# hangxu0304/DeepReduce

Measured on NVIDIA H100. Metric: ResNet-50 images/sec (whole job, device-timed, max over ranks), higher is better.
Workload: dtype bf16

## Files before the change

deepreduce_b200/models/resnet.py:

```python
from __future__ import annotations

import torch.nn as nn
import torch.nn.functional as F

from .fused_bn import bn_add_relu, bn_bn_add_relu, bn_relu, bn_relu_maxpool


class _BasicCifar(nn.Module):
    def __init__(self, inp, out, stride):
        super().__init__()
        self.conv1 = nn.Conv2d(inp, out, 3, stride, 1, bias=False)
        self.bn1 = nn.BatchNorm2d(out)
        self.conv2 = nn.Conv2d(out, out, 3, 1, 1, bias=False)
        self.bn2 = nn.BatchNorm2d(out)
        self.pad = None
        if stride != 1 or inp != out:
            self.pad = (out - inp, stride)

    def forward(self, x):
        y = F.relu(self.bn1(self.conv1(x)))
        y = self.bn2(self.conv2(y))
        if self.pad is not None:
            extra, s = self.pad
            x = F.pad(x[:, :, ::s, ::s], (0, 0, 0, 0, extra // 2, extra - extra // 2))
# ... 41 lines not shown
            self.downsample = nn.Sequential(nn.Conv2d(inp, out, 1, stride, bias=False), nn.BatchNorm2d(out))

    def forward(self, x, skip=None, fork=False):
        skip = x if skip is None else skip
        xd = None if self.downsample is None else self.downsample[0](skip)
        y = bn_relu(self.conv1(x), self.bn1)
        y = bn_relu(self.conv2(y), self.bn2)
        y = self.conv3(y)
        if xd is None:
            return bn_add_relu(y, self.bn3, skip, fork=fork)
        o = bn_bn_add_relu(y, self.bn3, xd, self.downsample[1])
        return (o, None) if fork else o


class ResNet(nn.Module):
    def __init__(self, blocks=(3, 4, 6, 3), num_classes: int = 1000):
        super().__init__()
        self.conv1 = nn.Conv2d(3, 64, 7, 2, 3, bias=False)
        self.bn1 = nn.BatchNorm2d(64)
        self.maxpool = nn.MaxPool2d(3, 2, 1)
        stages, inp = [], 64
        for i, (n, width) in enumerate(zip(blocks, (64, 128, 256, 512))):
            for j in range(n):
                stride = 2 if (j == 0 and i > 0) else 1
                stages.append(_Bottleneck(inp, width, stride, downsample=(j == 0)))
                inp = width * 4
        self.layers = nn.Sequential(*stages)
        self.fc = nn.Linear(inp, num_classes)
        for m in self.modules():
            if isinstance(m, nn.Conv2d):
                nn.init.kaiming_normal_(m.weight, mode="fan_out", nonlinearity="relu")

    def forward(self, x):
        x, skip = bn_relu_maxpool(self.conv1(x), self.bn1, self.maxpool), None
        for blk in self.layers:
            x, skip = blk(x, skip, fork=True)
        x = F.adaptive_avg_pool2d(x, 1).flatten(1)
        return self.fc(x)


def resnet50(num_classes: int = 1000) -> ResNet:
    return ResNet((3, 4, 6, 3), num_classes)
```

deepreduce_b200/ops/csrc/binding.cpp:

```cpp
#include <ATen/cuda/CUDAContext.h>
#include <c10/cuda/CUDAGuard.h>
#include <c10/cuda/CUDAStream.h>
#include <torch/extension.h>

#include <condition_variable>
#include <deque>
#include <mutex>
#include <thread>

#include "ops.h"

namespace py = pybind11;
using dr::EngineParams;

#define CHECK_CUDA_T(x) TORCH_CHECK((x).is_cuda() && (x).is_contiguous(), #x " must be a contiguous CUDA tensor")

static cudaStream_t cur_stream() { return at::cuda::getCurrentCUDAStream().stream(); }

static void check_last(const char* what) {
  cudaError_t e = cudaGetLastError();
  TORCH_CHECK(e == cudaSuccess, what, ": ", cudaGetErrorString(e));
}

static torch::Tensor bloom_insert(torch::Tensor idx, int64_t k, int64_t m_bits, int64_t seed) {
  CHECK_CUDA_T(idx);
  TORCH_CHECK(idx.scalar_type() == torch::kInt64, "idx must be int64");
  c10::cuda::CUDAGuard g(idx.device());
  const int64_t n_words = (m_bits + 31) / 32;
  auto words = torch::zeros({n_words}, idx.options().dtype(torch::kInt32));
  dr::launch_bloom_insert(idx.data_ptr<int64_t>(), idx.numel(), (uint32_t*)words.data_ptr<int32_t>(), (uint32_t)k,
                          (uint32_t)m_bits, (uint32_t)seed, cur_stream());
  check_last("bloom_insert");
  return words;
}

static torch::Tensor bloom_select(torch::Tensor words, int64_t d, int64_t limit, int64_t k, int64_t m_bits, int64_t seed) {
  CHECK_CUDA_T(words);
  c10::cuda::CUDAGuard g(words.device());
  const int64_t n_tiles = (d + dr::kTile - 1) / dr::kTile;
// ... 178 lines not shown

static torch::Tensor u8_to_nhwc_norm(torch::Tensor in, std::vector<double> mean, std::vector<double> stdv) {
  CHECK_CUDA_T(in);
  TORCH_CHECK(in.scalar_type() == torch::kUInt8 && in.size(-1) == 3, "expect uint8 [...,3] NHWC");
  c10::cuda::CUDAGuard g(in.device());
  auto out = torch::empty(in.sizes(), in.options().dtype(torch::kBFloat16));
  float m[3] = {(float)mean[0], (float)mean[1], (float)mean[2]};
  float s[3] = {(float)(1.0 / stdv[0]), (float)(1.0 / stdv[1]), (float)(1.0 / stdv[2])};
  dr::launch_u8_to_nhwc_norm(in.data_ptr<uint8_t>(), out.data_ptr(), in.numel() / 3, m, s, cur_stream());
  check_last("u8_to_nhwc_norm");
  return out;
}

namespace at::native {
struct Var;
template <typename scalar_t, typename VarTransform>
void batch_norm_stats_channels_last_cuda_template(const at::Tensor& out_mean, const at::Tensor& out_invstd,
                                                   const at::Tensor& input, double epsilon);
}

static void check_bn_input(const torch::Tensor& x) {
  TORCH_CHECK(x.is_cuda() && x.scalar_type() == torch::kBFloat16 && x.dim() == 4 && x.stride(1) == 1 &&
                  x.is_contiguous(at::MemoryFormat::ChannelsLast),
              "bn: x must be a channels_last bf16 CUDA tensor");
  TORCH_CHECK(x.size(1) % 8 == 0 && x.size(1) <= 8192, "bn: channels must be a multiple of 8, at most 8192");
  TORCH_CHECK(x.numel() < std::numeric_limits<int32_t>::max(), "bn: tensor too large for 32-bit indexing");
}

static void check_chan(const torch::Tensor& t, int64_t C, const char* what) {
  TORCH_CHECK(t.is_cuda() && t.scalar_type() == torch::kFloat32 && t.is_contiguous() && t.numel() == C, "bn: ", what,
              " must be a contiguous float32 CUDA tensor of C elements");
}

static std::vector<torch::Tensor> bn_stats(torch::Tensor x, torch::Tensor running_mean, torch::Tensor running_var,
                                           double momentum, double eps, bool torch_kernel) {
  check_bn_input(x);
  const int64_t C = x.size(1);
  check_chan(running_mean, C, "running_mean");
  check_chan(running_var, C, "running_var");
  const int64_t N = x.numel() / C;
  TORCH_CHECK(N > 1, "bn: expected more than 1 value per channel when training");
  c10::cuda::CUDAGuard g(x.device());
  auto opts = x.options().dtype(torch::kFloat32);
  auto mean = torch::empty({C}, opts), invstd = torch::empty({C}, opts);
  const float bessel = static_cast<float>(static_cast<double>(N) / static_cast<double>(N - 1));
  int block_y = 0, grid_y = 0;
  dr::bn_row_tree(N, (int)C, &block_y, &grid_y);
  cudaError_t e;
  if (!torch_kernel && (int64_t)block_y * grid_y <= N) {
    auto staging = grid_y > 1 ? torch::empty({(2 * C + 1) * grid_y}, opts) : torch::Tensor();
    const dr::BnStats s{x.data_ptr(), mean.data_ptr<float>(), invstd.data_ptr<float>(), running_mean.data_ptr<float>(),
                        running_var.data_ptr<float>(), grid_y > 1 ? staging.data_ptr<float>() : nullptr,
                        (float)momentum, bessel, (float)eps};
    e = dr::launch_bn_stats(s, N, (int)C, cur_stream());
  } else {
    at::native::batch_norm_stats_channels_last_cuda_template<c10::BFloat16, at::native::Var>(mean, invstd, x, eps);
    e = dr::launch_bn_update_stats(mean.data_ptr<float>(), invstd.data_ptr<float>(), running_mean.data_ptr<float>(),
                                   running_var.data_ptr<float>(), (int)C, (float)momentum, bessel, (float)eps,
                                   cur_stream());
  }
  TORCH_CHECK(e == cudaSuccess, "bn_stats: ", cudaGetErrorString(e));
  return {mean, invstd};
}

static dr::BnParams bn_params(const std::vector<torch::Tensor>& p, int64_t C) {
  TORCH_CHECK(p.size() == 4, "bn: expected (mean, invstd, weight, bias)");
  const char* names[4] = {"mean", "invstd", "weight", "bias"};
  for (int i = 0; i < 4; ++i) check_chan(p[i], C, names[i]);
  return {p[0].data_ptr<float>(), p[1].data_ptr<float>(), p[2].data_ptr<float>(), p[3].data_ptr<float>()};
}

static void check_like_x(const torch::Tensor& t, const torch::Tensor& x, const char* what) {
  TORCH_CHECK(t.sizes() == x.sizes() && t.strides() == x.strides() && t.scalar_type() == torch::kBFloat16 &&
                  t.device() == x.device(),
              "bn: ", what, " must match x in shape, layout, dtype and device");
}

static std::vector<torch::Tensor> bn_apply(int64_t mode, torch::Tensor x, std::vector<torch::Tensor> p,
                                           c10::optional<torch::Tensor> z, std::vector<torch::Tensor> pz) {
  check_bn_input(x);
  const int64_t C = x.size(1);
  const dr::BnParams px = bn_params(p, C);
  dr::BnParams pzz{};
  const void* zp = nullptr;
  if (mode != 0) {
// ... 360 lines not shown
```

deepreduce_b200/ops/csrc/bn.cu:

```cuda
#include <cuda_bf16.h>

#include <algorithm>

#include "common.cuh"
#include "ops.h"

namespace dr {

namespace {

constexpr int kVec = 8;
constexpr int kApplyThreads = 256;
constexpr int kReduceThreads = 128;

struct ChanParams {
  float m[kVec], inv[kVec], w[kVec], b[kVec];
};

__device__ __forceinline__ void load8(const float* __restrict__ p, float* d) {
  const float4 a = __ldg(reinterpret_cast<const float4*>(p));
  const float4 b = __ldg(reinterpret_cast<const float4*>(p) + 1);
  d[0] = a.x; d[1] = a.y; d[2] = a.z; d[3] = a.w;
  d[4] = b.x; d[5] = b.y; d[6] = b.z; d[7] = b.w;
}
// ... 36 lines not shown
  ChanParams a;
  load_params(px, c, a);
  ChanParams d;
  if (kMode == 2) load_params(pz, c, d);
  const int64_t step = (int64_t)gridDim.x * rows_per_cta;
#pragma unroll 2
  for (int64_t r = (int64_t)blockIdx.x * rows_per_cta + rsub; r < rows; r += step) {
    const int64_t off = r * C + c;
    const uint4 vx = *reinterpret_cast<const uint4*>(x + off);
    uint4 vz = make_uint4(0, 0, 0, 0);
    if (kMode != 0) vz = *reinterpret_cast<const uint4*>(z + off);
    const __nv_bfloat16* hx = reinterpret_cast<const __nv_bfloat16*>(&vx);
    const __nv_bfloat16* hz = reinterpret_cast<const __nv_bfloat16*>(&vz);
    uint4 vo;
    __nv_bfloat16* ho = reinterpret_cast<__nv_bfloat16*>(&vo);
    unsigned bits = 0;
#pragma unroll
    for (int i = 0; i < kVec; ++i) {
      __nv_bfloat16 y = __float2bfloat16_rn(bn_elem(__bfloat162float(hx[i]), a.m[i], a.inv[i], a.w[i], a.b[i]));
      if (kMode != 0) {
        const __nv_bfloat16 s = kMode == 1 ? hz[i]
                                           : __float2bfloat16_rn(bn_elem(__bfloat162float(hz[i]), d.m[i], d.inv[i], d.w[i], d.b[i]));
        y = __float2bfloat16_rn(__fadd_rn(__bfloat162float(y), __bfloat162float(s)));
      }
      ho[i] = relu_bf16(y);
      bits |= (__bfloat162float(ho[i]) <= 0.f ? 0u : 1u) << i;
    }
    *reinterpret_cast<uint4*>(out + off) = vo;
    mask[r * groups + c / kVec] = (uint8_t)bits;
  }
}


__global__ void __launch_bounds__(kApplyThreads) bn_apply_pool_kernel(const __nv_bfloat16* __restrict__ x, BnParams px,
                                                                      __nv_bfloat16* __restrict__ out,
                                                                      uint8_t* __restrict__ codes, int64_t orows,
                                                                      PoolGeom pg, int C) {
  const int groups = C / kVec;
  const int rows_per_cta = blockDim.x / groups;
  const int rsub = threadIdx.x / groups;
  if (rsub >= rows_per_cta) return;
  const int c = (threadIdx.x % groups) * kVec;
  ChanParams a;
  load_params(px, c, a);
  const int64_t step = (int64_t)gridDim.x * rows_per_cta;
  for (int64_t r = (int64_t)blockIdx.x * rows_per_cta + rsub; r < orows; r += step) {
    const int ow = (int)(r % pg.Wo);
    const int64_t t = r / pg.Wo;
    const int oh = (int)(t % pg.Ho);
    const int64_t n = t / pg.Ho;
    const int h0 = 2 * oh - 1, w0 = 2 * ow - 1;
    uint4 v[9];
#pragma unroll
    for (int k = 0; k < 9; ++k) {
      const int ih = h0 + k / 3, iw = w0 + k % 3;
      v[k] = ih >= 0 && ih < pg.H && iw >= 0 && iw < pg.W
                 ? *reinterpret_cast<const uint4*>(x + ((n * pg.H + ih) * pg.W + iw) * C + c)
                 : uint4{};
    }
    __nv_bfloat16 best[kVec];
    unsigned slot[kVec];
#pragma unroll
    for (int i = 0; i < kVec; ++i) {
      best[i] = __float2bfloat16_rn(-INFINITY);
      slot[i] = 0;
    }
#pragma unroll
    for (int k = 0; k < 9; ++k) {
      const int ih = h0 + k / 3, iw = w0 + k % 3;
      if (ih < 0 || ih >= pg.H || iw < 0 || iw >= pg.W) continue;
      const __nv_bfloat16* hx = reinterpret_cast<const __nv_bfloat16*>(&v[k]);
#pragma unroll
      for (int i = 0; i < kVec; ++i) {
        const __nv_bfloat16 y = relu_bf16(__float2bfloat16_rn(bn_elem(__bfloat162float(hx[i]), a.m[i], a.inv[i], a.w[i], a.b[i])));
        const float fy = __bfloat162float(y);
        if (fy > __bfloat162float(best[i]) || isnan(fy)) {
          best[i] = y;
          slot[i] = k;
        }
      }
    }
    uint4 vo;
    __nv_bfloat16* ho = reinterpret_cast<__nv_bfloat16*>(&vo);
    uint2 vc;
    uint8_t* hc = reinterpret_cast<uint8_t*>(&vc);
#pragma unroll
    for (int i = 0; i < kVec; ++i) {
      ho[i] = best[i];
      hc[i] = (uint8_t)(slot[i] | (__bfloat162float(best[i]) <= 0.f ? 0u : 0x80u));
    }
    *reinterpret_cast<uint4*>(out + r * C + c) = vo;
    *reinterpret_cast<uint2*>(codes + r * C + c) = vc;
  }
}

struct PoolGather {
  uint4 g[4];
  uint2 code[4];
  int off;
  int nh, nw;
  int sh, sw;
};

__device__ __forceinline__ void pool_gather_codes(PoolGather& q, const uint8_t* __restrict__ codes, const PoolGeom& pg,
                                                  int row, int C, int c, bool valid) {
  const int w = row % pg.W, t = row / pg.W, h = t % pg.H, n = t / pg.H;
  const int ph = h >> 1, pw = w >> 1;
  q.nh = valid ? min((h + 1) / 2 + 1, pg.Ho) - ph : 0;
  q.nw = valid ? min((w + 1) / 2 + 1, pg.Wo) - pw : 0;
  q.sh = h - 2 * ph + 1;
  q.sw = w - 2 * pw + 1;
  q.off = ((n * pg.Ho + ph) * pg.Wo + pw) * C + c;
#pragma unroll
  for (int k = 0; k < 4; ++k) {
    const int a = k >> 1, b = k & 1;
    q.code[k] = a < q.nh && b < q.nw ? *reinterpret_cast<const uint2*>(codes + q.off + (a * pg.Wo + b) * C) : uint2{};
  }
}

template <bool kTwo>
__device__ __forceinline__ void pool_gather_grads(PoolGather& q, const __nv_bfloat16* __restrict__ gp,
                                                  const __nv_bfloat16* __restrict__ gp2, const PoolGeom& pg, int C) {
#pragma unroll
  for (int k = 0; k < 4; ++k) {
    const int a = k >> 1, b = k & 1;
    const bool in = a < q.nh && b < q.nw;
    const int off = q.off + (a * pg.Wo + b) * C;
    q.g[k] = in ? *reinterpret_cast<const uint4*>(gp + off) : uint4{};
    if (kTwo && in) q.g[k] = add_bf16x8(q.g[k], *reinterpret_cast<const uint4*>(gp2 + off));
  }
}

__device__ __forceinline__ void pool_gather_resolve(const PoolGather& q, uint4& g, unsigned& bits) {
  __nv_bfloat16* hg = reinterpret_cast<__nv_bfloat16*>(&g);
  const bool single = q.nh == 1 && q.nw == 1;
  bits = 0;
#pragma unroll
  for (int i = 0; i < kVec; ++i) {
    float s = 0.f;
    __nv_bfloat16 one = __float2bfloat16_rn(0.f);
    unsigned bit = 0;
#pragma unroll
    for (int k = 0; k < 4; ++k) {
      const int a = k >> 1, b = k & 1;
      const unsigned code = (reinterpret_cast<const uint8_t*>(&q.code[k]))[i];
      if (a < q.nh && b < q.nw && (int)(code & 0x7fu) == (q.sh - 2 * a) * 3 + (q.sw - 2 * b)) {
        const __nv_bfloat16 v = (reinterpret_cast<const __nv_bfloat16*>(&q.g[k]))[i];
        s = __fadd_rn(s, __bfloat162float(v));
        one = v;
        bit = code >> 7;
      }
    }
    hg[i] = single ? one : __float2bfloat16_rn(s);
    bits |= bit << i;
  }
}

template <bool kTwo>
__global__ void __launch_bounds__(kApplyThreads) bn_pool_grad_kernel(const __nv_bfloat16* __restrict__ gp,
                                                                     const __nv_bfloat16* __restrict__ gp2,
                                                                     const uint8_t* __restrict__ codes,
                                                                     __nv_bfloat16* __restrict__ g, PoolGeom pg,
                                                                     int64_t rows, int C) {
  const int groups = C / kVec;
  const int rows_per_cta = blockDim.x / groups;
  const int rsub = threadIdx.x / groups;
  if (rsub >= rows_per_cta) return;
  const int c = (threadIdx.x % groups) * kVec;
  const int64_t step = (int64_t)gridDim.x * rows_per_cta;
#pragma unroll 2
  for (int64_t r = (int64_t)blockIdx.x * rows_per_cta + rsub; r < rows; r += step) {
    PoolGather q;
    pool_gather_codes(q, codes, pg, (int)r, C, c, true);
    pool_gather_grads<kTwo>(q, gp, gp2, pg, C);
    uint4 v;
    unsigned bits;
    pool_gather_resolve(q, v, bits);
    __nv_bfloat16* hv = reinterpret_cast<__nv_bfloat16*>(&v);
#pragma unroll
    for (int i = 0; i < kVec; ++i)
      if (!((bits >> i) & 1u)) hv[i] = __float2bfloat16_rn(0.f);
    *reinterpret_cast<uint4*>(g + r * C + c) = v;
  }
}

struct RowTree {
  int block_y, grid_y;
  __host__ __device__ int S() const { return block_y * grid_y; }
  __host__ __device__ int loops(int rows) const { return 1 + (rows - 1) / (S() * kLoads); }
  static constexpr int kLoads = 4;
};

constexpr int kStatsThreads = 256;

__device__ __forceinline__ void welford_update(float x, float inv, float valid, float& mean, float& m2n) {
  const float d0 = __fsub_rn(x, mean);
  mean = __fmaf_rn(d0, inv, mean);
  const float d1 = __fsub_rn(x, mean);
  m2n = __fmaf_rn(__fmul_rn(d0, d1), valid, m2n);
}

template <int kN, bool kFuseNew>
__device__ __forceinline__ void welford_merge(int& n, float* mean, float* m2n, int n_new, const float* mean_new,
                                              const float* m2n_new) {
  const float fn = (float)n, fn_new = (float)n_new;
  const float factor = __frcp_rn((float)max(1, n + n_new));
#pragma unroll
  for (int i = 0; i < kN; ++i) {
    const float d = __fsub_rn(mean[i], mean_new[i]);
    const float s = kFuseNew ? __fmaf_rn(mean_new[i], fn_new, __fmul_rn(mean[i], fn))
                             : __fmaf_rn(mean[i], fn, __fmul_rn(mean_new[i], fn_new));
    mean[i] = __fmul_rn(s, factor);
    const float u = __fmul_rn(__fmul_rn(__fmul_rn(d, d), fn_new), fn);
    m2n[i] = __fadd_rn(m2n[i], __fmaf_rn(u, factor, m2n_new[i]));
  }
// ... 3 lines not shown
template <int kN>
struct WelfordSlots {
  float* mean; float* m2n; int* count;
  __device__ WelfordSlots(float* sh, int slots)
      : mean(sh), m2n(sh + slots * kN), count(reinterpret_cast<int*>(sh + 2 * slots * kN)) {}
  __device__ void put(int s, int n, const float* m, const float* q) const {
#pragma unroll
    for (int i = 0; i < kN; ++i) { mean[s * kN + i] = m[i]; m2n[s * kN + i] = q[i]; }
    count[s] = n;
  }
  template <bool kFuseNew>
  __device__ void merge_from(int s, int& n, float* m, float* q) const {
    float mn[kN], qn[kN];
#pragma unroll
    for (int i = 0; i < kN; ++i) { mn[i] = mean[s * kN + i]; qn[i] = m2n[s * kN + i]; }
    welford_merge<kN, kFuseNew>(n, m, q, count[s], mn, qn);
  }
  static size_t bytes(int slots) { return (size_t)slots * (2 * kN * sizeof(float) + sizeof(int)); }
};

template <int kN>
__device__ __forceinline__ void welford_tree_over_y(const WelfordSlots<kN>& sl, bool part, int y, int block_y, int base,
                                                    int stride, int& n, float* mean, float* m2n) {
  for (int off = block_y / 2; off > 0; off >>= 1) {
    if (part && y < 2 * off) sl.put(base + y * stride, n, mean, m2n);
    __syncthreads();
    if (part && y < off) sl.template merge_from<false>(base + (y + off) * stride, n, mean, m2n);
    __syncthreads();
  }
}

struct StatsOut {
  float* mean; float* invstd; float* running_mean; float* running_var;
  float* st_mean; float* st_m2n; int* st_count;
  float momentum, bessel, eps;
};

__device__ __forceinline__ void stats_store(const StatsOut& o, int c, int n, float mean, float m2n) {
  const float var = __fdiv_rn(m2n, (float)n);
  const float keep = __fsub_rn(1.f, o.momentum);
  o.mean[c] = mean;
  o.invstd[c] = rsqrtf(__fadd_rn(var, o.eps));
  o.running_mean[c] = __fmaf_rn(mean, o.momentum, __fmul_rn(o.running_mean[c], keep));
  o.running_var[c] = __fmaf_rn(__fmul_rn(var, o.bessel), o.momentum, __fmul_rn(o.running_var[c], keep));
}

__global__ void __launch_bounds__(kStatsThreads) bn_stats_kernel(const __nv_bfloat16* __restrict__ x, StatsOut o,
                                                                 RowTree t, int rows, int C) {
  constexpr int L = RowTree::kLoads;
  constexpr int kAhead = 4;
  extern __shared__ float sh[];
  const int gpc = blockDim.x / (L * t.block_y);
  const int g = threadIdx.x % gpc, j = (threadIdx.x / gpc) % L, y = threadIdx.x / (gpc * L);
  const int group = blockIdx.x * gpc + g;
  const bool live = group * kVec < C;
  const int c = live ? group * kVec : 0;
  const int S = t.S();
  const int n_loops = t.loops(rows);
  const int r0 = blockIdx.y * t.block_y + y + j * S;
  const int rstep = L * S;
  float mean[kVec], m2n[kVec];
#pragma unroll
  for (int i = 0; i < kVec; ++i) mean[i] = m2n[i] = 0.f;
  int n = 0;
  auto load = [&](uint4* b, int i0) {
#pragma unroll
    for (int u = 0; u < kAhead; ++u) {
      const int r = r0 + (i0 + u) * rstep;
      b[u] = live && i0 + u < n_loops && r < rows ? *reinterpret_cast<const uint4*>(x + (size_t)r * C + c) : uint4{};
    }
  };
  uint4 cur[kAhead];
  load(cur, 0);
  for (int i0 = 0; i0 < n_loops; i0 += kAhead) {
    uint4 nxt[kAhead];
    load(nxt, i0 + kAhead);
#pragma unroll
    for (int u = 0; u < kAhead; ++u) {
      const int i = i0 + u;
      if (i >= n_loops) break;
      const bool valid = r0 + i * rstep < rows;
      const float inv = valid ? __frcp_rn((float)(i + 1)) : 0.f;
      const float fv = valid ? 1.f : 0.f;
      n += valid;
      const __nv_bfloat16* hx = reinterpret_cast<const __nv_bfloat16*>(&cur[u]);
#pragma unroll
      for (int k = 0; k < kVec; ++k) welford_update(__bfloat162float(hx[k]), inv, fv, mean[k], m2n[k]);
    }
#pragma unroll
    for (int u = 0; u < kAhead; ++u) cur[u] = nxt[u];
  }
  const WelfordSlots<kVec> sl(sh, blockDim.x);
  sl.put(threadIdx.x, n, mean, m2n);
  __syncthreads();
  if (j == 0) {
#pragma unroll
    for (int a = 1; a < L; ++a) sl.merge_from<true>(threadIdx.x + a * gpc, n, mean, m2n);
  }
  __syncthreads();
  welford_tree_over_y<kVec>(sl, j == 0, y, t.block_y, g, gpc * L, n, mean, m2n);
  if (j != 0 || y != 0 || !live) return;
  if (t.grid_y == 1) {
#pragma unroll
    for (int i = 0; i < kVec; ++i) stats_store(o, c + i, n, mean[i], m2n[i]);
    return;
  }
#pragma unroll
  for (int i = 0; i < kVec; ++i) {
    o.st_mean[(size_t)blockIdx.y * C + c + i] = mean[i];
    o.st_m2n[(size_t)blockIdx.y * C + c + i] = m2n[i];
  }
  if (group == 0) o.st_count[blockIdx.y] = n;
}

__global__ void bn_stats_finalize_kernel(StatsOut o, RowTree t, int C) {
  extern __shared__ float sh[];
  const int cols = blockDim.x / t.block_y;
  const int col = threadIdx.x % cols, y = threadIdx.x / cols;
  const int c = blockIdx.x * cols + col;
  int n = 0;
  float mean = 0.f, m2n = 0.f;
  if (c < C)
    for (int b = y; b < t.grid_y; b += t.block_y) {
      const float mb = o.st_mean[(size_t)b * C + c], qb = o.st_m2n[(size_t)b * C + c];
      welford_merge<1, false>(n, &mean, &m2n, o.st_count[b], &mb, &qb);
    }
  const WelfordSlots<1> sl(sh, blockDim.x);
  welford_tree_over_y<1>(sl, true, y, t.block_y, col, cols, n, &mean, &m2n);
  if (y == 0 && c < C) stats_store(o, c, n, mean, m2n);
}


template <int kN>
__device__ __forceinline__ void tree_over_y(float* v, float* sh, int y, int n, int col, int width) {
  for (int off = n / 2; off > 0; off >>= 1) {
#pragma unroll
    for (int i = 0; i < kN; ++i) sh[y * width + col + i] = v[i];
    __syncthreads();
    if (y < off) {
#pragma unroll
      for (int i = 0; i < kN; ++i) v[i] = __fadd_rn(v[i], sh[(y + off) * width + col + i]);
    }
    __syncthreads();
  }
}

struct BwdOut {
  float* sums;
  float* dw; float* db; float* dwz; float* dbz;
  float* staging;
};

__device__ __forceinline__ void bwd_store(const BwdOut& o, int k, int c, int C, float v, const float* invstd,
                                         const float* invstd_z) {
  o.sums[k * C + c] = v;
  if (k == 0) {
    o.db[c] = v;
    if (o.dbz) o.dbz[c] = v;
  } else if (k == 1) {
    o.dw[c] = __fmul_rn(v, invstd[c]);
  } else {
    o.dwz[c] = __fmul_rn(v, invstd_z[c]);
// ... 195 lines not shown
      if (kMode == 2) hd[i] = elemt(g, __bfloat162float(hz[i]), q, i, norm);
    }
    *reinterpret_cast<uint4*>(dx + off) = vo;
    if (kMode == 2) *reinterpret_cast<uint4*>(dz + off) = vd;
  }
}

__global__ void bn_update_stats_kernel(const float* __restrict__ mean, float* __restrict__ var_invstd,
                                       float* __restrict__ running_mean, float* __restrict__ running_var, int C,
                                       float momentum, float bessel, float eps) {
  const int c = blockIdx.x * blockDim.x + threadIdx.x;
  if (c >= C) return;
  const float m = mean[c], v = var_invstd[c];
  const float unbiased_var = v * bessel;
  running_mean[c] = m * momentum + (1 - momentum) * running_mean[c];
  running_var[c] = unbiased_var * momentum + (1 - momentum) * running_var[c];
  var_invstd[c] = rsqrtf(v + eps);
}

template <typename K>
cudaError_t rows_grid(K kernel, int64_t rows, int C, int& grid, int& threads) {
  const int groups = C / kVec;
  const int rows_per_cta = groups >= kApplyThreads ? 1 : kApplyThreads / groups;
  threads = groups * rows_per_cta;
  int per_sm = 0;
  cudaError_t e = cudaOccupancyMaxActiveBlocksPerMultiprocessor(&per_sm, kernel, threads, 0);
  if (e != cudaSuccess) return e;
  int64_t g = (rows + rows_per_cta - 1) / rows_per_cta;
  const int64_t cap = (int64_t)(per_sm > 0 ? per_sm : 1) * sm_count();
  grid = (int)(g > cap ? cap : g);
  return cudaSuccess;
}

template <int kMode>
cudaError_t launch_apply(const void* x, const BnParams& px, const void* z, const BnParams& pz, void* out, void* mask,
                         int64_t rows, int C, cudaStream_t st) {
  if (rows == 0) return cudaSuccess;
  int grid = 0, threads = 0;
  cudaError_t e = rows_grid(bn_apply_kernel<kMode>, rows, C, grid, threads);
  if (e != cudaSuccess) return e;
  count_launch();
  bn_apply_kernel<kMode><<<grid, threads, 0, st>>>(reinterpret_cast<const __nv_bfloat16*>(x), px,
                                                   reinterpret_cast<const __nv_bfloat16*>(z), pz,
                                                   reinterpret_cast<__nv_bfloat16*>(out),
                                                   reinterpret_cast<uint8_t*>(mask), rows, C);
  return cudaGetLastError();
}

int last_pow2(unsigned n) {
  n |= n >> 1; n |= n >> 2; n |= n >> 4; n |= n >> 8; n |= n >> 16;
  return std::max<int>(1, (int)(n - (n >> 1)));
}

RowTree row_tree(int rows, int C) {
  const int block_x = std::min(last_pow2((unsigned)C), 32);
  const int block_y = std::min(last_pow2((unsigned)((rows + 15) / 16)), 512 / block_x);
  int grid_y = std::min((rows + block_y * 16 - 1) / (block_y * 16), 128);
  if (grid_y < 8) grid_y = 1;
  return {block_y, grid_y};
}

template <int kMode, bool kTwo>
cudaError_t launch_bwd_reduce(const BnBwd& b, const RowTree& t, const BwdOut& o, int rows, int C, cudaStream_t st) {
  const int groups = C / kVec;
  const int gpc = std::min(groups, std::max(1, kReduceThreads / t.block_y));
  const dim3 grid((groups + gpc - 1) / gpc, t.grid_y);
  const int threads = gpc * t.block_y;
  count_launch();
  bn_bwd_reduce_kernel<kMode, kTwo><<<grid, threads, threads * kVec * sizeof(float), st>>>(
      reinterpret_cast<const __nv_bfloat16*>(b.go), reinterpret_cast<const __nv_bfloat16*>(b.go2), b.mask,
      reinterpret_cast<const __nv_bfloat16*>(b.x), b.px.mean, b.px.invstd, reinterpret_cast<const __nv_bfloat16*>(b.z),
      b.pz.mean, b.pz.invstd, reinterpret_cast<__nv_bfloat16*>(b.g), o, t, rows, C);
  return cudaGetLastError();
}

template <int kMode, bool kTwo>
cudaError_t launch_bwd_elemt(const BnBwd& b, const ElemtArgs& a, int64_t rows, int C, cudaStream_t st) {
  int grid = 0, threads = 0;
  cudaError_t e = rows_grid(bn_bwd_elemt_kernel<kMode, kTwo>, rows, C, grid, threads);
  if (e != cudaSuccess) return e;
  const float norm = (float)(1.0 / (double)rows);
  count_launch();
  bn_bwd_elemt_kernel<kMode, kTwo><<<grid, threads, 0, st>>>(
      reinterpret_cast<const __nv_bfloat16*>(kMode == 1 || kMode == 3 ? b.g : b.go),
      reinterpret_cast<const __nv_bfloat16*>(b.go2), b.mask, reinterpret_cast<const __nv_bfloat16*>(b.x),
      reinterpret_cast<const __nv_bfloat16*>(b.z), a, reinterpret_cast<__nv_bfloat16*>(b.dx),
      reinterpret_cast<__nv_bfloat16*>(b.dz), norm, rows, C);
  return cudaGetLastError();
}

template <int kMode, bool kTwo>
cudaError_t launch_backward(const BnBwd& b, int64_t rows64, int C, cudaStream_t st) {
  const int rows = (int)rows64;
  const RowTree t = row_tree(rows, C);
  const BwdOut o{b.sums, b.dw, b.db, b.dwz, b.dbz, b.staging};
  cudaError_t e;
  if (kMode == 3) {
    int grid = 0, threads = 0;
    e = rows_grid(bn_pool_grad_kernel<kTwo>, rows64, C, grid, threads);
    if (e != cudaSuccess) return e;
    count_launch();
    bn_pool_grad_kernel<kTwo><<<grid, threads, 0, st>>>(reinterpret_cast<const __nv_bfloat16*>(b.go),
                                                        reinterpret_cast<const __nv_bfloat16*>(b.go2), b.mask,
                                                        reinterpret_cast<__nv_bfloat16*>(b.g), b.pool, rows64, C);
    e = cudaGetLastError();
    if (e != cudaSuccess) return e;
  }
  BnBwd bb = b;
  if (kMode == 3) bb.go = b.g;
  e = launch_bwd_reduce<kMode, kTwo && kMode != 3>(bb, t, o, rows, C, st);
  if (e != cudaSuccess) return e;
  if (t.grid_y > 1) {
    const int cols = std::max(1, 512 / t.block_y);
    const int threads = cols * t.block_y;
    count_launch();
    bn_bwd_finalize_kernel<<<(C + cols - 1) / cols, threads, threads * sizeof(float), st>>>(
        o, t, kMode == 2 ? 3 : 2, C, b.px.invstd, b.pz.invstd);
    e = cudaGetLastError();
    if (e != cudaSuccess) return e;
  }
  const ElemtArgs a{b.px.mean, b.px.invstd, b.px.weight, b.sums, b.pz.mean, b.pz.invstd, b.pz.weight};
  return launch_bwd_elemt<kMode, kTwo && kMode == 2>(b, a, rows64, C, st);
}

cudaError_t launch_stats(const BnStats& s, int rows, int C, cudaStream_t st) {
  const RowTree t = row_tree(rows, C);
  const int grid_y = t.grid_y;
  const StatsOut o{s.mean, s.invstd, s.running_mean, s.running_var,
                   s.staging, s.staging + (size_t)grid_y * C, reinterpret_cast<int*>(s.staging + 2 * (size_t)grid_y * C),
                   s.momentum, s.bessel, s.eps};
  const int groups = C / kVec;
  const int gpc = std::min(groups, std::max(1, kStatsThreads / (RowTree::kLoads * t.block_y)));
  const int threads = gpc * RowTree::kLoads * t.block_y;
  count_launch();
  bn_stats_kernel<<<dim3((groups + gpc - 1) / gpc, grid_y), threads, WelfordSlots<kVec>::bytes(threads), st>>>(
      reinterpret_cast<const __nv_bfloat16*>(s.x), o, t, rows, C);
  cudaError_t e = cudaGetLastError();
  if (e != cudaSuccess || grid_y == 1) return e;
  const int cols = std::max(1, 512 / t.block_y);
  const int fthreads = cols * t.block_y;
  count_launch();
  bn_stats_finalize_kernel<<<(C + cols - 1) / cols, fthreads, WelfordSlots<1>::bytes(fthreads), st>>>(o, t, C);
  return cudaGetLastError();
}

}

void bn_row_tree(int64_t rows, int C, int* block_y, int* grid_y) {
  const RowTree t = row_tree((int)rows, C);
  *block_y = t.block_y;
  *grid_y = t.grid_y;
}

cudaError_t launch_bn_backward(int mode, const BnBwd& b, int64_t rows, int C, cudaStream_t st) {
  if (rows == 0) return cudaSuccess;
  const bool two = b.go2 != nullptr;
  switch (mode) {
    case 0: return two ? cudaErrorInvalidValue : launch_backward<0, false>(b, rows, C, st);
    case 1: return two ? launch_backward<1, true>(b, rows, C, st) : launch_backward<1, false>(b, rows, C, st);
    case 2: return two ? launch_backward<2, true>(b, rows, C, st) : launch_backward<2, false>(b, rows, C, st);
    case 3: return two ? launch_backward<3, true>(b, rows, C, st) : launch_backward<3, false>(b, rows, C, st);
    default: return cudaErrorInvalidValue;
  }
}

cudaError_t launch_bn_stats(const BnStats& s, int64_t rows, int C, cudaStream_t st) {
  if (rows == 0) return cudaSuccess;
  return launch_stats(s, (int)rows, C, st);
}

cudaError_t launch_bn_update_stats(const float* mean, float* var_invstd, float* running_mean, float* running_var, int C,
                                   float momentum, float bessel, float eps, cudaStream_t st) {
  count_launch();
  bn_update_stats_kernel<<<(C + 255) / 256, 256, 0, st>>>(mean, var_invstd, running_mean, running_var, C, momentum,
                                                          bessel, eps);
  return cudaGetLastError();
}

cudaError_t launch_bn_apply(int mode, const void* x, const BnParams& px, const void* z, const BnParams& pz, void* out,
                            void* mask, int64_t rows, int C, cudaStream_t st) {
  switch (mode) {
    case 0: return launch_apply<0>(x, px, z, pz, out, mask, rows, C, st);
    case 1: return launch_apply<1>(x, px, z, pz, out, mask, rows, C, st);
    case 2: return launch_apply<2>(x, px, z, pz, out, mask, rows, C, st);
    default: return cudaErrorInvalidValue;
  }
}

cudaError_t launch_bn_apply_pool(const void* x, const BnParams& px, void* out, void* codes, int N, const PoolGeom& pg,
                                 int C, cudaStream_t st) {
  const int64_t orows = (int64_t)N * pg.Ho * pg.Wo;
  if (orows == 0) return cudaSuccess;
  int grid = 0, threads = 0;
  cudaError_t e = rows_grid(bn_apply_pool_kernel, orows, C, grid, threads);
  if (e != cudaSuccess) return e;
  count_launch();
  bn_apply_pool_kernel<<<grid, threads, 0, st>>>(reinterpret_cast<const __nv_bfloat16*>(x), px,
                                                 reinterpret_cast<__nv_bfloat16*>(out),
                                                 reinterpret_cast<uint8_t*>(codes), orows, pg, C);
  return cudaGetLastError();
}

}
```

deepreduce_b200/ops/csrc/ops.h:

```cpp
#pragma once
#include <cuda_runtime.h>
#include <stdint.h>

#include "plan.h"

namespace dr {

int engine_max_grid(int blocks_per_sm, int dyn_smem_bytes);
cudaError_t engine_launch(const EngineParams& P, int grid, int blocks_per_sm, int dyn_smem_bytes, cudaStream_t stream);
void count_launch(int n);
long long launch_count();

void launch_bloom_insert(const int64_t* idx, int64_t n, uint32_t* filter, uint32_t n_hash, uint32_t m_bits,
                         uint32_t seed, cudaStream_t st);
void launch_bloom_count(const uint32_t* filter, uint32_t d, uint32_t n_hash, uint32_t m_bits, uint32_t seed,
                        uint32_t* tile_counts, uint32_t* tile_excl, cudaStream_t st);
void launch_bloom_emit(const uint32_t* filter, uint32_t d, uint32_t n_hash, uint32_t m_bits, uint32_t seed,
                       const uint32_t* tile_excl, int64_t* out, uint32_t limit, cudaStream_t st);
void launch_qsgd_encode(const float* v, int64_t K, int bucket, int q, uint32_t seed, void* lvl, bool i16, float* norms,
                        cudaStream_t st);
void launch_qsgd_decode(const void* lvl, bool i16, const float* norms, int64_t K, int bucket, int q, float* out,
                        cudaStream_t st);
void launch_pack_bits(const int64_t* vals, int64_t n, int bits, uint32_t* out, int64_t n_words, cudaStream_t st);
void launch_unpack_bits(const uint32_t* in, int64_t n_words, int64_t n, int bits, int64_t* out, cudaStream_t st);
void launch_polyfit_fit(const float* y, const int* seg_off, const int* seg_len, int n_seg, int degree, float* coeffs,
                        cudaStream_t st);
void launch_polyfit_eval(const float* coeffs, const int* seg_off, const int* seg_len, int n_seg, int degree,
                         int64_t total, float* out, cudaStream_t st);
cudaError_t launch_conflict_sets_pick(const uint32_t* set_off, const uint32_t* members, uint32_t* last, uint32_t n_sets, uint32_t n_pos,
                                      uint32_t K, uint32_t pseed, uint32_t* chosen_out, cudaStream_t st);
void launch_dexp_fit(const float* y, int64_t K, double* out_abpq, cudaStream_t st);
void launch_bp128_widths(const int64_t* idx, int64_t n, uint32_t* widths, cudaStream_t st);
void launch_bp128_pack(const int64_t* idx, int64_t n, const uint32_t* widths, const int64_t* word_off, uint32_t* out,
                       cudaStream_t st);
void launch_bp128_unpack(const uint32_t* in, int64_t n, int64_t* word_off, int64_t* deltas, cudaStream_t st);
void launch_rle_count(const int64_t* idx, int64_t n, uint32_t* counts, uint32_t* excl, cudaStream_t st);
void launch_rle_runs(const int64_t* idx, int64_t n, const uint32_t* excl, int64_t* start_pos, int64_t* end_pos,
                     int64_t n_runs, int64_t d, int64_t* runs, cudaStream_t st);
void launch_rle_expand(const int64_t* ones_excl, const int64_t* run_start, int64_t n_runs, int64_t total, int64_t* out,
                       cudaStream_t st);

struct ArenaHandle { unsigned char bytes[64]; };
void* arena_alloc(size_t bytes);
void arena_free(void* p);
ArenaHandle arena_export(void* p);
void* arena_import(const ArenaHandle& h);
void arena_close(void* p);
int arena_enable_peer_access(const int* devices, int n);
void launch_u8_to_nhwc_norm(const uint8_t* in, void* out_bf16, int64_t n_pix, const float* mean, const float* inv_std,
                            cudaStream_t st);

struct BnParams { const float* mean; const float* invstd; const float* weight; const float* bias; };
void bn_row_tree(int64_t rows, int C, int* block_y, int* grid_y);
struct BnStats {
  const void* x;
  float* mean; float* invstd; float* running_mean; float* running_var;
  float* staging;
  float momentum, bessel, eps;
};
cudaError_t launch_bn_stats(const BnStats& s, int64_t rows, int C, cudaStream_t st);
cudaError_t launch_bn_update_stats(const float* mean, float* var_invstd, float* running_mean, float* running_var, int C,
                                   float momentum, float bessel, float eps, cudaStream_t st);
cudaError_t launch_bn_apply(int mode, const void* x, const BnParams& px, const void* z, const BnParams& pz, void* out,
                            void* mask, int64_t rows, int C, cudaStream_t st);
struct PoolGeom { int H, W, Ho, Wo; };
cudaError_t launch_bn_apply_pool(const void* x, const BnParams& px, void* out, void* codes, int N, const PoolGeom& pg,
                                 int C, cudaStream_t st);
struct BnBwd {
  const void* go; const void* go2; const uint8_t* mask; const void* x; const void* z;
  BnParams px, pz;
  void* dx; void* dz; void* g;
  float* sums; float* staging; float* dw; float* db; float* dwz; float* dbz;
  PoolGeom pool;
};
cudaError_t launch_bn_backward(int mode, const BnBwd& b, int64_t rows, int C, cudaStream_t st);

}
```

Baseline: 6178.

## Fuse BN stats finalize via last-block reduction and rework maxpool kernels

```diff
diff --git a/deepreduce_b200/models/resnet.py b/deepreduce_b200/models/resnet.py
--- a/deepreduce_b200/models/resnet.py
+++ b/deepreduce_b200/models/resnet.py
@@ -97,7 +97,7 @@
                 nn.init.kaiming_normal_(m.weight, mode="fan_out", nonlinearity="relu")
 
     def forward(self, x):
-        x, skip = bn_relu_maxpool(self.conv1(x), self.bn1, self.maxpool), None
+        x, skip = bn_relu_maxpool(self.conv1(x), self.bn1, self.maxpool, fork=True)
         for blk in self.layers:
             x, skip = blk(x, skip, fork=True)
         x = F.adaptive_avg_pool2d(x, 1).flatten(1)
diff --git a/deepreduce_b200/ops/csrc/binding.cpp b/deepreduce_b200/ops/csrc/binding.cpp
--- a/deepreduce_b200/ops/csrc/binding.cpp
+++ b/deepreduce_b200/ops/csrc/binding.cpp
@@ -5,6 +5,7 @@
 
 #include <condition_variable>
 #include <deque>
+#include <map>
 #include <mutex>
 #include <thread>
 
@@ -249,6 +250,20 @@
               " must be a contiguous float32 CUDA tensor of C elements");
 }
 
+static unsigned* bn_stats_arrivals(int device, cudaStream_t st) {
+  static std::mutex mu;
+  static std::map<std::pair<int, cudaStream_t>, unsigned*> sets;
+  std::lock_guard<std::mutex> lock(mu);
+  unsigned*& p = sets[{device, st}];
+  if (p == nullptr) {
+    void* q = nullptr;
+    C10_CUDA_CHECK(cudaMalloc(&q, dr::kBnStatsArrivals * sizeof(unsigned)));
+    C10_CUDA_CHECK(cudaMemsetAsync(q, 0, dr::kBnStatsArrivals * sizeof(unsigned), st));
+    p = static_cast<unsigned*>(q);
+  }
+  return p;
+}
+
 static std::vector<torch::Tensor> bn_stats(torch::Tensor x, torch::Tensor running_mean, torch::Tensor running_var,
                                            double momentum, double eps, bool torch_kernel) {
   check_bn_input(x);
@@ -265,9 +280,10 @@
   dr::bn_row_tree(N, (int)C, &block_y, &grid_y);
   cudaError_t e;
   if (!torch_kernel && (int64_t)block_y * grid_y <= N) {
-    auto staging = grid_y > 1 ? torch::empty({(2 * C + 1) * grid_y}, opts) : torch::Tensor();
+    auto staging = grid_y > 1 ? torch::empty({(2 * C + C / 8) * grid_y}, opts) : torch::Tensor();
     const dr::BnStats s{x.data_ptr(), mean.data_ptr<float>(), invstd.data_ptr<float>(), running_mean.data_ptr<float>(),
                         running_var.data_ptr<float>(), grid_y > 1 ? staging.data_ptr<float>() : nullptr,
+                        grid_y > 1 ? bn_stats_arrivals(x.get_device(), cur_stream()) : nullptr,
                         (float)momentum, bessel, (float)eps};
     e = dr::launch_bn_stats(s, N, (int)C, cur_stream());
   } else {
diff --git a/deepreduce_b200/ops/csrc/bn.cu b/deepreduce_b200/ops/csrc/bn.cu
--- a/deepreduce_b200/ops/csrc/bn.cu
+++ b/deepreduce_b200/ops/csrc/bn.cu
@@ -92,32 +92,89 @@
 }
 
 
-__global__ void __launch_bounds__(kApplyThreads) bn_apply_pool_kernel(const __nv_bfloat16* __restrict__ x, BnParams px,
-                                                                      __nv_bfloat16* __restrict__ out,
-                                                                      uint8_t* __restrict__ codes, int64_t orows,
-                                                                      PoolGeom pg, int C) {
+constexpr int kPoolThreads = 128;
+constexpr int kPoolWalk = 8;
+
+struct PoolWalk {
+  int64_t n;
+  int oh, ow0, ow1, c;
+};
+
+__device__ __forceinline__ bool pool_walk(const PoolGeom& pg, int N, int C, PoolWalk& w) {
   const int groups = C / kVec;
-  const int rows_per_cta = blockDim.x / groups;
-  const int rsub = threadIdx.x / groups;
-  if (rsub >= rows_per_cta) return;
-  const int c = (threadIdx.x % groups) * kVec;
+  const int segs = (pg.Wo + kPoolWalk - 1) / kPoolWalk;
+  const int64_t t = (int64_t)blockIdx.x * blockDim.x + threadIdx.x;
+  const int64_t task = t / groups;
+  if (task >= (int64_t)N * pg.Ho * segs) return false;
+  w.c = (int)(t % groups) * kVec;
+  const int seg = (int)(task % segs);
+  const int64_t row = task / segs;
+  w.oh = (int)(row % pg.Ho);
+  w.n = row / pg.Ho;
+  w.ow0 = seg * kPoolWalk;
+  w.ow1 = min(w.ow0 + kPoolWalk, pg.Wo);
+  return true;
+}
+
+__device__ __forceinline__ uint4 bn_relu8(const uint4& v, const ChanParams& a) {
+  uint4 r;
+  const __nv_bfloat16* hx = reinterpret_cast<const __nv_bfloat16*>(&v);
+  __nv_bfloat16* hr = reinterpret_cast<__nv_bfloat16*>(&r);
+#pragma unroll
+  for (int i = 0; i < kVec; ++i)
+    hr[i] = relu_bf16(__float2bfloat16_rn(bn_elem(__bfloat162float(hx[i]), a.m[i], a.inv[i], a.w[i], a.b[i])));
+  return r;
+}
+
+__global__ void __launch_bounds__(kPoolThreads) bn_apply_pool_kernel(const __nv_bfloat16* __restrict__ x, BnParams px,
+                                                                     __nv_bfloat16* __restrict__ out,
+                                                                     uint8_t* __restrict__ codes, int N, PoolGeom pg,
+                                                                     int C) {
+  PoolWalk w;
+  if (!pool_walk(pg, N, C, w)) return;
   ChanParams a;
-  load_params(px, c, a);
-  const int64_t step = (int64_t)gridDim.x * rows_per_cta;
-  for (int64_t r = (int64_t)blockIdx.x * rows_per_cta + rsub; r < orows; r += step) {
-    const int ow = (int)(r % pg.Wo);
-    const int64_t t = r / pg.Wo;
-    const int oh = (int)(t % pg.Ho);
-    const int64_t n = t / pg.Ho;
-    const int h0 = 2 * oh - 1, w0 = 2 * ow - 1;
-    uint4 v[9];
-#pragma unroll
-    for (int k = 0; k < 9; ++k) {
-      const int ih = h0 + k / 3, iw = w0 + k % 3;
-      v[k] = ih >= 0 && ih < pg.H && iw >= 0 && iw < pg.W
-                 ? *reinterpret_cast<const uint4*>(x + ((n * pg.H + ih) * pg.W + iw) * C + c)
-                 : uint4{};
-    }
+  load_params(px, w.c, a);
+  bool row_in[3];
+  const __nv_bfloat16* xrow[3];
+#pragma unroll
+  for (int kh = 0; kh < 3; ++kh) {
+    const int ih = 2 * w.oh - 1 + kh;
+    row_in[kh] = ih >= 0 && ih < pg.H;
+    xrow[kh] = x + ((w.n * pg.H + (row_in[kh] ? ih : 0)) * pg.W) * C + w.c;
+  }
+  auto load = [&](int kh, int iw) {
+    return row_in[kh] && iw >= 0 && iw < pg.W ? *reinterpret_cast<const uint4*>(xrow[kh] + (int64_t)iw * C) : uint4{};
+  };
+  uint4 left[3];
+  uint4 nxt[3][2];
+#pragma unroll
+  for (int kh = 0; kh < 3; ++kh) {
+    left[kh] = bn_relu8(load(kh, 2 * w.ow0 - 1), a);
+    nxt[kh][0] = load(kh, 2 * w.ow0);
+    nxt[kh][1] = load(kh, 2 * w.ow0 + 1);
+  }
+  int64_t o = ((w.n * pg.Ho + w.oh) * pg.Wo + w.ow0) * C + w.c;
+  for (int ow = w.ow0; ow < w.ow1; ++ow, o += C) {
+    uint4 v[3][3];
+#pragma unroll
+    for (int kh = 0; kh < 3; ++kh) {
+      v[kh][0] = left[kh];
+      v[kh][1] = nxt[kh][0];
+      v[kh][2] = nxt[kh][1];
+    }
+    if (ow + 1 < w.ow1)
+#pragma unroll
+      for (int kh = 0; kh < 3; ++kh) {
+        nxt[kh][0] = load(kh, 2 * ow + 2);
+        nxt[kh][1] = load(kh, 2 * ow + 3);
+      }
+#pragma unroll
+    for (int kh = 0; kh < 3; ++kh) {
+      v[kh][1] = bn_relu8(v[kh][1], a);
+      v[kh][2] = bn_relu8(v[kh][2], a);
+      left[kh] = v[kh][2];
+    }
+    const bool col_in[3] = {ow > 0, true, 2 * ow + 1 < pg.W};
     __nv_bfloat16 best[kVec];
     unsigned slot[kVec];
 #pragma unroll
@@ -127,15 +184,13 @@
     }
 #pragma unroll
     for (int k = 0; k < 9; ++k) {
-      const int ih = h0 + k / 3, iw = w0 + k % 3;
-      if (ih < 0 || ih >= pg.H || iw < 0 || iw >= pg.W) continue;
-      const __nv_bfloat16* hx = reinterpret_cast<const __nv_bfloat16*>(&v[k]);
+      if (!row_in[k / 3] || !col_in[k % 3]) continue;
+      const __nv_bfloat16* hy = reinterpret_cast<const __nv_bfloat16*>(&v[k / 3][k % 3]);
 #pragma unroll
       for (int i = 0; i < kVec; ++i) {
-        const __nv_bfloat16 y = relu_bf16(__float2bfloat16_rn(bn_elem(__bfloat162float(hx[i]), a.m[i], a.inv[i], a.w[i], a.b[i])));
-        const float fy = __bfloat162float(y);
+        const float fy = __bfloat162float(hy[i]);
         if (fy > __bfloat162float(best[i]) || isnan(fy)) {
-          best[i] = y;
+          best[i] = hy[i];
           slot[i] = k;
         }
       }
@@ -149,47 +204,17 @@
       ho[i] = best[i];
       hc[i] = (uint8_t)(slot[i] | (__bfloat162float(best[i]) <= 0.f ? 0u : 0x80u));
     }
-    *reinterpret_cast<uint4*>(out + r * C + c) = vo;
-    *reinterpret_cast<uint2*>(codes + r * C + c) = vc;
+    *reinterpret_cast<uint4*>(out + o) = vo;
+    *reinterpret_cast<uint2*>(codes + o) = vc;
   }
 }
 
 struct PoolGather {
   uint4 g[4];
   uint2 code[4];
-  int off;
   int nh, nw;
   int sh, sw;
 };
-
-__device__ __forceinline__ void pool_gather_codes(PoolGather& q, const uint8_t* __restrict__ codes, const PoolGeom& pg,
-                                                  int row, int C, int c, bool valid) {
-  const int w = row % pg.W, t = row / pg.W, h = t % pg.H, n = t / pg.H;
-  const int ph = h >> 1, pw = w >> 1;
-  q.nh = valid ? min((h + 1) / 2 + 1, pg.Ho) - ph : 0;
-  q.nw = valid ? min((w + 1) / 2 + 1, pg.Wo) - pw : 0;
-  q.sh = h - 2 * ph + 1;
-  q.sw = w - 2 * pw + 1;
-  q.off = ((n * pg.Ho + ph) * pg.Wo + pw) * C + c;
-#pragma unroll
-  for (int k = 0; k < 4; ++k) {
-    const int a = k >> 1, b = k & 1;
-    q.code[k] = a < q.nh && b < q.nw ? *reinterpret_cast<const uint2*>(codes + q.off + (a * pg.Wo + b) * C) : uint2{};
-  }
-}
-
-template <bool kTwo>
-__device__ __forceinline__ void pool_gather_grads(PoolGather& q, const __nv_bfloat16* __restrict__ gp,
-                                                  const __nv_bfloat16* __restrict__ gp2, const PoolGeom& pg, int C) {
-#pragma unroll
-  for (int k = 0; k < 4; ++k) {
-    const int a = k >> 1, b = k & 1;
-    const bool in = a < q.nh && b < q.nw;
-    const int off = q.off + (a * pg.Wo + b) * C;
-    q.g[k] = in ? *reinterpret_cast<const uint4*>(gp + off) : uint4{};
-    if (kTwo && in) q.g[k] = add_bf16x8(q.g[k], *reinterpret_cast<const uint4*>(gp2 + off));
-  }
-}
 
 __device__ __forceinline__ void pool_gather_resolve(const PoolGather& q, uint4& g, unsigned& bits) {
   __nv_bfloat16* hg = reinterpret_cast<__nv_bfloat16*>(&g);
@@ -217,30 +242,63 @@
 }
 
 template <bool kTwo>
-__global__ void __launch_bounds__(kApplyThreads) bn_pool_grad_kernel(const __nv_bfloat16* __restrict__ gp,
-                                                                     const __nv_bfloat16* __restrict__ gp2,
-                                                                     const uint8_t* __restrict__ codes,
-                                                                     __nv_bfloat16* __restrict__ g, PoolGeom pg,
-                                                                     int64_t rows, int C) {
-  const int groups = C / kVec;
-  const int rows_per_cta = blockDim.x / groups;
-  const int rsub = threadIdx.x / groups;
-  if (rsub >= rows_per_cta) return;
-  const int c = (threadIdx.x % groups) * kVec;
-  const int64_t step = (int64_t)gridDim.x * rows_per_cta;
-#pragma unroll 2
-  for (int64_t r = (int64_t)blockIdx.x * rows_per_cta + rsub; r < rows; r += step) {
-    PoolGather q;
-    pool_gather_codes(q, codes, pg, (int)r, C, c, true);
-    pool_gather_grads<kTwo>(q, gp, gp2, pg, C);
-    uint4 v;
-    unsigned bits;
-    pool_gather_resolve(q, v, bits);
-    __nv_bfloat16* hv = reinterpret_cast<__nv_bfloat16*>(&v);
-#pragma unroll
-    for (int i = 0; i < kVec; ++i)
-      if (!((bits >> i) & 1u)) hv[i] = __float2bfloat16_rn(0.f);
-    *reinterpret_cast<uint4*>(g + r * C + c) = v;
+__global__ void __launch_bounds__(kPoolThreads) bn_pool_grad_kernel(const __nv_bfloat16* __restrict__ gp,
+                                                                    const __nv_bfloat16* __restrict__ gp2,
+                                                                    const uint8_t* __restrict__ codes,
+                                                                    __nv_bfloat16* __restrict__ g, int N, PoolGeom pg,
+                                                                    int C) {
+  PoolWalk w;
+  if (!pool_walk(pg, N, C, w)) return;
+  const int nh = min(2, pg.Ho - w.oh);
+  const int64_t prow = (w.n * pg.Ho + w.oh) * pg.Wo;
+  auto load = [&](int a, int ow, uint4& gv, uint2& cv) {
+    if (a < nh && ow < pg.Wo) {
+      const int64_t off = (prow + (int64_t)a * pg.Wo + ow) * C + w.c;
+      gv = *reinterpret_cast<const uint4*>(gp + off);
+      if (kTwo) gv = add_bf16x8(gv, *reinterpret_cast<const uint4*>(gp2 + off));
+      cv = *reinterpret_cast<const uint2*>(codes + off);
+    } else {
+      gv = uint4{};
+      cv = uint2{};
+    }
+  };
+  uint4 gl[2];
+  uint2 cl[2];
+  load(0, w.ow0, gl[0], cl[0]);
+  load(1, w.ow0, gl[1], cl[1]);
+  for (int ow = w.ow0; ow < w.ow1; ++ow) {
+    uint4 gr[2];
+    uint2 cr[2];
+    load(0, ow + 1, gr[0], cr[0]);
+    load(1, ow + 1, gr[1], cr[1]);
+    const int nw = min(2, pg.Wo - ow);
+#pragma unroll
+    for (int a = 0; a < 2; ++a) {
+      const int h = 2 * w.oh + a;
+      if (h >= pg.H) break;
+#pragma unroll
+      for (int b = 0; b < 2; ++b) {
+        const int iw = 2 * ow + b;
+        if (iw >= pg.W) break;
+        PoolGather q;
+        q.g[0] = gl[0]; q.g[1] = gr[0]; q.g[2] = gl[1]; q.g[3] = gr[1];
+        q.code[0] = cl[0]; q.code[1] = cr[0]; q.code[2] = cl[1]; q.code[3] = cr[1];
+        q.nh = a == 0 ? 1 : nh;
+        q.nw = b == 0 ? 1 : nw;
+        q.sh = a + 1;
+        q.sw = b + 1;
+        uint4 v;
+        unsigned bits;
+        pool_gather_resolve(q, v, bits);
+        __nv_bfloat16* hv = reinterpret_cast<__nv_bfloat16*>(&v);
+#pragma unroll
+        for (int i = 0; i < kVec; ++i)
+          if (!((bits >> i) & 1u)) hv[i] = __float2bfloat16_rn(0.f);
+        *reinterpret_cast<uint4*>(g + ((w.n * pg.H + h) * pg.W + iw) * C + w.c) = v;
+      }
+    }
+    gl[0] = gr[0]; gl[1] = gr[1];
+    cl[0] = cr[0]; cl[1] = cr[1];
   }
 }
 
@@ -310,7 +368,7 @@
 
 struct StatsOut {
   float* mean; float* invstd; float* running_mean; float* running_var;
-  float* st_mean; float* st_m2n; int* st_count;
+  float* st_mean; float* st_m2n; int* st_count; unsigned* arrivals;
   float momentum, bessel, eps;
 };
 
@@ -323,7 +381,44 @@
   o.running_var[c] = __fmaf_rn(__fmul_rn(var, o.bessel), o.momentum, __fmul_rn(o.running_var[c], keep));
 }
 
-__global__ void __launch_bounds__(kStatsThreads) bn_stats_kernel(const __nv_bfloat16* __restrict__ x, StatsOut o,
+__device__ __forceinline__ void stats_cross_block(const StatsOut& o, const RowTree& t, float* sh, int C, int cb_c0) {
+  constexpr int kRows = 8;
+  const int cols = blockDim.x / t.block_y;
+  const int col = threadIdx.x % cols, y = threadIdx.x / cols;
+  const int c = cb_c0 + 2 * col;
+  const bool live = c < C;
+  int n = 0;
+  float mean[2] = {0.f, 0.f}, m2n[2] = {0.f, 0.f};
+  if (live)
+    for (int b0 = y; b0 < t.grid_y; b0 += kRows * t.block_y) {
+      float2 mb[kRows], qb[kRows];
+      int nb[kRows];
+#pragma unroll
+      for (int u = 0; u < kRows; ++u) {
+        const int b = b0 + u * t.block_y;
+        if (b < t.grid_y) {
+          const size_t off = (size_t)b * C + c;
+          mb[u] = __ldcg(reinterpret_cast<const float2*>(o.st_mean + off));
+          qb[u] = __ldcg(reinterpret_cast<const float2*>(o.st_m2n + off));
+          nb[u] = __ldcg(o.st_count + (size_t)blockIdx.x * t.grid_y + b);
+        }
+      }
+#pragma unroll
+      for (int u = 0; u < kRows; ++u) {
+        if (b0 + u * t.block_y >= t.grid_y) break;
+        const float mbv[2] = {mb[u].x, mb[u].y}, qbv[2] = {qb[u].x, qb[u].y};
+        welford_merge<2, false>(n, mean, m2n, nb[u], mbv, qbv);
+      }
+    }
+  const WelfordSlots<2> sl(sh, blockDim.x);
+  welford_tree_over_y<2>(sl, true, y, t.block_y, col, cols, n, mean, m2n);
+  if (y == 0 && live) {
+    stats_store(o, c, n, mean[0], m2n[0]);
+    stats_store(o, c + 1, n, mean[1], m2n[1]);
+  }
+}
+
+__global__ void __launch_bounds__(kStatsThreads, 768 / kStatsThreads) bn_stats_kernel(const __nv_bfloat16* __restrict__ x, StatsOut o,
                                                                  RowTree t, int rows, int C) {
   constexpr int L = RowTree::kLoads;
   constexpr int kAhead = 4;
@@ -377,35 +472,32 @@
   }
   __syncthreads();
   welford_tree_over_y<kVec>(sl, j == 0, y, t.block_y, g, gpc * L, n, mean, m2n);
-  if (j != 0 || y != 0 || !live) return;
+  const bool head = j == 0 && y == 0 && live;
   if (t.grid_y == 1) {
-#pragma unroll
-    for (int i = 0; i < kVec; ++i) stats_store(o, c + i, n, mean[i], m2n[i]);
+    if (head)
+#pragma unroll
+      for (int i = 0; i < kVec; ++i) stats_store(o, c + i, n, mean[i], m2n[i]);
     return;
   }
-#pragma unroll
-  for (int i = 0; i < kVec; ++i) {
-    o.st_mean[(size_t)blockIdx.y * C + c + i] = mean[i];
-    o.st_m2n[(size_t)blockIdx.y * C + c + i] = m2n[i];
-  }
-  if (group == 0) o.st_count[blockIdx.y] = n;
-}
-
-__global__ void bn_stats_finalize_kernel(StatsOut o, RowTree t, int C) {
-  extern __shared__ float sh[];
-  const int cols = blockDim.x / t.block_y;
-  const int col = threadIdx.x % cols, y = threadIdx.x / cols;
-  const int c = blockIdx.x * cols + col;
-  int n = 0;
-  float mean = 0.f, m2n = 0.f;
-  if (c < C)
-    for (int b = y; b < t.grid_y; b += t.block_y) {
-      const float mb = o.st_mean[(size_t)b * C + c], qb = o.st_m2n[(size_t)b * C + c];
-      welford_merge<1, false>(n, &mean, &m2n, o.st_count[b], &mb, &qb);
-    }
-  const WelfordSlots<1> sl(sh, blockDim.x);
-  welford_tree_over_y<1>(sl, true, y, t.block_y, col, cols, n, &mean, &m2n);
-  if (y == 0 && c < C) stats_store(o, c, n, mean, m2n);
+  if (head) {
+#pragma unroll
+    for (int i = 0; i < kVec; ++i) {
+      o.st_mean[(size_t)blockIdx.y * C + c + i] = mean[i];
+      o.st_m2n[(size_t)blockIdx.y * C + c + i] = m2n[i];
+    }
+    if (g == 0) o.st_count[(size_t)blockIdx.x * t.grid_y + blockIdx.y] = n;
+    __threadfence();
+  }
+  __shared__ bool last;
+  __syncthreads();
+  if (threadIdx.x == 0) {
+    last = atomicAdd(o.arrivals + blockIdx.x, 1u) == (unsigned)t.grid_y - 1;
+    if (last) o.arrivals[blockIdx.x] = 0;
+  }
+  __syncthreads();
+  if (!last) return;
+  __threadfence();
+  stats_cross_block(o, t, sh, C, blockIdx.x * gpc * kVec);
 }
 
 
@@ -667,6 +759,11 @@
   return cudaSuccess;
 }
 
+unsigned pool_walk_grid(int N, const PoolGeom& pg, int C) {
+  const int64_t threads = (int64_t)N * pg.Ho * ((pg.Wo + kPoolWalk - 1) / kPoolWalk) * (C / kVec);
+  return (unsigned)((threads + kPoolThreads - 1) / kPoolThreads);
+}
+
 template <int kMode>
 cudaError_t launch_apply(const void* x, const BnParams& px, const void* z, const BnParams& pz, void* out, void* mask,
                          int64_t rows, int C, cudaStream_t st) {
@@ -731,13 +828,11 @@
   const BwdOut o{b.sums, b.dw, b.db, b.dwz, b.dbz, b.staging};
   cudaError_t e;
   if (kMode == 3) {
-    int grid = 0, threads = 0;
-    e = rows_grid(bn_pool_grad_kernel<kTwo>, rows64, C, grid, threads);
-    if (e != cudaSuccess) return e;
+    const int N = (int)(rows64 / ((int64_t)b.pool.H * b.pool.W));
     count_launch();
-    bn_pool_grad_kernel<kTwo><<<grid, threads, 0, st>>>(reinterpret_cast<const __nv_bfloat16*>(b.go),
-                                                        reinterpret_cast<const __nv_bfloat16*>(b.go2), b.mask,
-                                                        reinterpret_cast<__nv_bfloat16*>(b.g), b.pool, rows64, C);
+    bn_pool_grad_kernel<kTwo><<<pool_walk_grid(N, b.pool, C), kPoolThreads, 0, st>>>(
+        reinterpret_cast<const __nv_bfloat16*>(b.go), reinterpret_cast<const __nv_bfloat16*>(b.go2), b.mask,
+        reinterpret_cast<__nv_bfloat16*>(b.g), N, b.pool, C);
     e = cudaGetLastError();
     if (e != cudaSuccess) return e;
   }
@@ -763,19 +858,13 @@
   const int grid_y = t.grid_y;
   const StatsOut o{s.mean, s.invstd, s.running_mean, s.running_var,
                    s.staging, s.staging + (size_t)grid_y * C, reinterpret_cast<int*>(s.staging + 2 * (size_t)grid_y * C),
-                   s.momentum, s.bessel, s.eps};
+                   s.arrivals, s.momentum, s.bessel, s.eps};
   const int groups = C / kVec;
   const int gpc = std::min(groups, std::max(1, kStatsThreads / (RowTree::kLoads * t.block_y)));
   const int threads = gpc * RowTree::kLoads * t.block_y;
   count_launch();
   bn_stats_kernel<<<dim3((groups + gpc - 1) / gpc, grid_y), threads, WelfordSlots<kVec>::bytes(threads), st>>>(
       reinterpret_cast<const __nv_bfloat16*>(s.x), o, t, rows, C);
-  cudaError_t e = cudaGetLastError();
-  if (e != cudaSuccess || grid_y == 1) return e;
-  const int cols = std::max(1, 512 / t.block_y);
-  const int fthreads = cols * t.block_y;
-  count_launch();
-  bn_stats_finalize_kernel<<<(C + cols - 1) / cols, fthreads, WelfordSlots<1>::bytes(fthreads), st>>>(o, t, C);
   return cudaGetLastError();
 }
 
@@ -824,15 +913,11 @@
 
 cudaError_t launch_bn_apply_pool(const void* x, const BnParams& px, void* out, void* codes, int N, const PoolGeom& pg,
                                  int C, cudaStream_t st) {
-  const int64_t orows = (int64_t)N * pg.Ho * pg.Wo;
-  if (orows == 0) return cudaSuccess;
-  int grid = 0, threads = 0;
-  cudaError_t e = rows_grid(bn_apply_pool_kernel, orows, C, grid, threads);
-  if (e != cudaSuccess) return e;
+  if ((int64_t)N * pg.Ho * pg.Wo == 0) return cudaSuccess;
   count_launch();
-  bn_apply_pool_kernel<<<grid, threads, 0, st>>>(reinterpret_cast<const __nv_bfloat16*>(x), px,
-                                                 reinterpret_cast<__nv_bfloat16*>(out),
-                                                 reinterpret_cast<uint8_t*>(codes), orows, pg, C);
+  bn_apply_pool_kernel<<<pool_walk_grid(N, pg, C), kPoolThreads, 0, st>>>(reinterpret_cast<const __nv_bfloat16*>(x), px,
+                                                                          reinterpret_cast<__nv_bfloat16*>(out),
+                                                                          reinterpret_cast<uint8_t*>(codes), N, pg, C);
   return cudaGetLastError();
 }
 
diff --git a/deepreduce_b200/ops/csrc/ops.h b/deepreduce_b200/ops/csrc/ops.h
--- a/deepreduce_b200/ops/csrc/ops.h
+++ b/deepreduce_b200/ops/csrc/ops.h
@@ -52,10 +52,12 @@
 
 struct BnParams { const float* mean; const float* invstd; const float* weight; const float* bias; };
 void bn_row_tree(int64_t rows, int C, int* block_y, int* grid_y);
+constexpr int kBnStatsArrivals = 8192 / 8;
 struct BnStats {
   const void* x;
   float* mean; float* invstd; float* running_mean; float* running_var;
   float* staging;
+  unsigned* arrivals;
   float momentum, bessel, eps;
 };
 cudaError_t launch_bn_stats(const BnStats& s, int64_t rows, int C, cudaStream_t st);
```

Result: faster. 6257, median of 6 (+1.3%).
